# MiNeves00/SR-GAN-FD

Hardware: AMD Instinct MI355X
Metric: SR training images/sec (128->512 x4, f16) (higher is better)
Workload: dtype f16; 1 GPU; BSRGAN RRDBNet x4 generator-only (L1), 23 RRDB, batch 32/GPU, 128->512; global_batch=32, num_rrdb=23, parallelism=dp1

## Files before the change

include/srganfd.h:

```cpp
#ifndef SRGANFD_H
#define SRGANFD_H
#include <stddef.h>
#include <stdint.h>
#ifdef __cplusplus
extern "C" {
#endif

#define SRGANFD_OK 0
#define SRGANFD_EINVAL (-1)
#define SRGANFD_EHIP (-2)
#define SRGANFD_ENOSPC (-3)

#define SRGANFD_BF16 0
#define SRGANFD_F32 1
#define SRGANFD_F16 2

#define SRGANFD_ACT_NONE 0
#define SRGANFD_ACT_LRELU 1
#define SRGANFD_ACT_RELU 2

const char* srganfd_last_error(void);
#define SRGANFD_ABI_VERSION 7
int srganfd_abi_version(void);
void srganfd_set_dry_run(int on);
// ... 26 lines not shown
  srganfd_view y2;
  int32_t out_classes, class_pad_step;
} srganfd_conv_args;

int srganfd_conv2d(const srganfd_conv_args* a, void* stream);
int srganfd_conv2d_describe(const srganfd_conv_args* a, char* out, size_t out_len);

int srganfd_dense_chain(const srganfd_conv_args* layers, int32_t n_layers, void* workspace, size_t workspace_bytes, void* stream);
int srganfd_dense_chain_check(const srganfd_conv_args* layers, int32_t n_layers);
size_t srganfd_dense_chain_workspace_bytes(void);

typedef struct {
  int64_t src_off;
  int64_t scale_off;
  int32_t co_src, ci_src;
  int32_t k_lo, k_len;
  int32_t co_off, ci_off;
  int32_t transposed;
  float scale;
} srganfd_pack_seg;

typedef struct {
  int64_t dst_off;
  int32_t dtype, ksize;
  int32_t k, n;
  int32_t nseg;
  int32_t layout;
  srganfd_pack_seg seg[5];
} srganfd_pack_job;

size_t srganfd_packed_bytes(int32_t dtype, int32_t ksize, int32_t k, int32_t n);
int srganfd_get_mfma16(void);
int srganfd_pack_layout(int32_t dtype, int32_t ksize, int32_t n);
int srganfd_pack_weights(const srganfd_pack_job* jobs_dev, int32_t njobs, int64_t max_elems,
                         const float* params, const float* scalars, void* packed, void* stream);

typedef struct {
  int32_t ci_lo, cin;
  int32_t co_lo, cout;
  int64_t dw_off;
  int64_t db_off;
  int32_t co_dst, ci_dst;
  float alpha;
  float beta;
  int64_t alpha_off;
} srganfd_wgrad_conv;

typedef struct {
  int32_t dtype;
  int32_t n, h_in, w_in, up, ksize, stride, pad, h_out, w_out;
  int32_t x_channels, dy_channels;
  int32_t nconv;
  int32_t splits;
} srganfd_wgrad_shape;

size_t srganfd_wgrad_plan_bytes(const srganfd_wgrad_shape* s, const srganfd_wgrad_conv* convs);
int srganfd_wgrad_plan_build(const srganfd_wgrad_shape* s, const srganfd_wgrad_conv* convs,
                             void* plan_host, size_t plan_bytes, size_t* workspace_bytes);
int srganfd_conv2d_wgrad(const void* plan_host, const void* plan_dev, srganfd_view x, srganfd_view dy,
                         float* grads, const float* scalars, void* workspace, size_t workspace_bytes,
                         void* stream);
typedef struct {
  const void* plan_host; const void* plan_dev;
  float* grads; const float* scalars; const void* workspace;
} srganfd_wgrad_reduce_job;
int srganfd_conv2d_wgrad_partial(const void* plan_host, const void* plan_dev, srganfd_view x, srganfd_view dy,
                                 void* workspace, size_t workspace_bytes, void* stream);
int srganfd_wgrad_reduce_batch(const srganfd_wgrad_reduce_job* jobs, int32_t njobs, void* stream);

int srganfd_nchw_to_nhwc(const float* src, int32_t n, int32_t c, int32_t h, int32_t w, srganfd_view dst,
                         int32_t dtype, int32_t cpad, const float* ch_mean, const float* ch_std, void* stream);
int srganfd_nhwc_to_nchw(srganfd_view src, int32_t dtype, int32_t n, int32_t c, int32_t h, int32_t w,
                         float* dst, int32_t clamp01, void* stream);
int srganfd_clamp_grad_to_nhwc(const float* dsr_nchw, srganfd_view pre_f32, int32_t n, int32_t c, int32_t h,
                               int32_t w, srganfd_view dst, int32_t dtype, int32_t cpad, void* stream);

int srganfd_resample(int32_t op, srganfd_view a, srganfd_view b, int32_t dtype, int32_t n, int32_t h,
                     int32_t w, int32_t c, void* stream);
int srganfd_resample_bwd_lrelu(srganfd_view dy, srganfd_view dx_raw, srganfd_view act, srganfd_view dx_masked,
                               int32_t dtype, int32_t n, int32_t h, int32_t w, int32_t c, float slope, void* stream);
int srganfd_lrelu_bwd(srganfd_view dy, srganfd_view act, srganfd_view skip, srganfd_view out, int32_t dtype,
                      int64_t npix, int32_t c, float slope, void* stream);
int srganfd_axpby(srganfd_view x, srganfd_view y, int32_t dtype, int64_t npix, int32_t c, float alpha,
                  float beta, void* stream);

#define SRGANFD_LOSS_WS_FLOATS 2049
int srganfd_l1_loss(const float* a, const float* b, int64_t numel, float weight, float* out,
                    int32_t accumulate, float* grad_a , float grad_scale,
                    const float* grad_scale_dev , float* workspace, void* stream);
int srganfd_l1_loss_views(srganfd_view a, srganfd_view b, int32_t dtype, int64_t npix, int32_t c,
                          int32_t relu_first, float weight, float* out, int32_t accumulate,
                          float* workspace, void* stream);
int srganfd_bce_logits(const float* logits, int64_t numel, float target, float weight, float* loss_out,
                       int32_t accumulate, float* sigmoid_mean_out , float* grad ,
                       float grad_scale, const float* grad_scale_dev , float* workspace, void* stream);
int srganfd_bce_logits_relativistic(const float* x, int64_t numel, const float* other, int64_t numel_other, float target, float weight,
                                    float* loss_out, int32_t accumulate, float* grad_x , int32_t accumulate_x,
                                    float* grad_other , int32_t accumulate_other, float grad_scale,
                                    const float* grad_scale_dev , float* workspace, void* stream);
int srganfd_sigmoid_of_mean(const float* logits, int64_t numel, float* out, float* workspace, void* stream);

int srganfd_spectral_norm(const float* w_orig, float* u, float* v, int32_t rows, int32_t cols,
                          int32_t training, float eps, float* sigma_out, float* inv_sigma_out,
                          float* workspace, void* stream);
#define SRGANFD_SN_BATCH 8
typedef struct srganfd_sn_job {
  const float* w_orig; float* u; float* v; float* sigma_out; float* inv_sigma_out; float* workspace;
  int32_t rows, cols;
} srganfd_sn_job;
int srganfd_spectral_norm_batch(const srganfd_sn_job* jobs, int32_t njobs, int32_t training, float eps, void* stream);
int srganfd_spectral_norm_grad(const float* g_weight, const float* w_orig, const float* u, const float* v,
                               const float* inv_sigma, float* dw_orig, int32_t rows, int32_t cols,
                               float beta, float* workspace, void* stream);
typedef struct srganfd_sn_grad_job {
  const float* g_weight; const float* w_orig; const float* u; const float* v; const float* inv_sigma;
  float* dw_orig; float* workspace;
  int32_t rows, cols;
} srganfd_sn_grad_job;
int srganfd_spectral_norm_grad_batch(const srganfd_sn_grad_job* jobs, int32_t njobs, float beta, void* stream);

int srganfd_adam_ema(float* param, const float* grad, float* exp_avg, float* exp_avg_sq, float* ema,
// ... 167 lines not shown
```

sr_gan_fd_amd/_abi.py:

```python
from __future__ import annotations

import ctypes as C
import os

_HERE = os.path.dirname(os.path.abspath(__file__))
LIB_PATH = os.environ.get("SRGANFD_LIB") or os.path.join(_HERE, "libsrganfd_hip.so")

HEADER = os.path.join(os.path.dirname(_HERE), "include", "srganfd.h")


_ABI_VERSION_BUILT = 7


def _header_abi_version() -> int:
    import re
    try:
        with open(HEADER) as f:
            m = re.search(r"^#define\s+SRGANFD_ABI_VERSION\s+(\d+)", f.read(), re.M)
    except OSError:
        return _ABI_VERSION_BUILT
    if not m:
        raise RuntimeError(f"{HEADER}: SRGANFD_ABI_VERSION not found")
    return int(m.group(1))

# ... 99 lines not shown
    ]


class LpipsTap(C.Structure):
    C_NAME = "srganfd_lpips_tap"
    _fields_ = [("maps", C.c_void_p), ("lin", C.c_void_p), ("h", C.c_int32), ("w", C.c_int32), ("c", C.c_int32), ("pad_", C.c_int32)]


class AttnArgs(C.Structure):
    C_NAME = "srganfd_attn_args"
    _fields_ = [
        ("dtype", C.c_int32), ("batch", C.c_int32), ("seq", C.c_int32), ("heads", C.c_int32), ("head_dim", C.c_int32), ("pad_", C.c_int32),
        ("qkv", C.c_void_p), ("out", C.c_void_p), ("lse", C.c_void_p), ("d_out", C.c_void_p), ("d_qkv", C.c_void_p), ("weights", C.c_void_p),
        ("workspace", C.c_void_p), ("workspace_bytes", C.c_size_t),
    ]


SYMBOLS = {
    "srganfd_last_error": (C.c_char_p, []),
    "srganfd_abi_version": (C.c_int, []),
    "srganfd_set_dry_run": (None, [C.c_int]),
    "srganfd_get_mfma16": (C.c_int, []),
    "srganfd_pack_layout": (C.c_int, [C.c_int32, C.c_int32, C.c_int32]),
    "srganfd_conv2d": (C.c_int, [C.POINTER(ConvArgs), C.c_void_p]),
    "srganfd_conv2d_describe": (C.c_int, [C.POINTER(ConvArgs), C.c_char_p, C.c_size_t]),
    "srganfd_dense_chain": (C.c_int, [C.POINTER(ConvArgs), C.c_int32, C.c_void_p, C.c_size_t, C.c_void_p]),
    "srganfd_dense_chain_check": (C.c_int, [C.POINTER(ConvArgs), C.c_int32]),
    "srganfd_dense_chain_workspace_bytes": (C.c_size_t, []),
    "srganfd_conv2d_thin_in": (C.c_int, [C.POINTER(ThinArgs), C.c_void_p]),
    "srganfd_conv2d_thin_out": (C.c_int, [C.POINTER(ThinArgs), C.c_void_p]),
    "srganfd_conv2d_thin_wgrad_workspace": (C.c_size_t, []),
    "srganfd_conv2d_thin_wgrad": (C.c_int, [C.POINTER(ThinArgs), C.c_void_p, C.c_void_p, C.c_void_p, C.c_size_t, C.c_void_p]),
    "srganfd_packed_bytes": (C.c_size_t, [C.c_int32, C.c_int32, C.c_int32, C.c_int32]),
    "srganfd_pack_weights": (C.c_int, [C.c_void_p, C.c_int32, C.c_int64, C.c_void_p, C.c_void_p, C.c_void_p, C.c_void_p]),
    "srganfd_wgrad_plan_bytes": (C.c_size_t, [C.POINTER(WgradShape), C.POINTER(WgradConv)]),
    "srganfd_wgrad_plan_build": (C.c_int, [C.POINTER(WgradShape), C.POINTER(WgradConv), C.c_void_p, C.c_size_t,
                                           C.POINTER(C.c_size_t)]),
    "srganfd_conv2d_wgrad_partial": (C.c_int, [C.c_void_p, C.c_void_p, View, View, C.c_void_p, C.c_size_t, C.c_void_p]),
    "srganfd_wgrad_reduce_batch": (C.c_int, [C.c_void_p, C.c_int32, C.c_void_p]),
    "srganfd_conv2d_wgrad": (C.c_int, [C.c_void_p, C.c_void_p, View, View, C.c_void_p, C.c_void_p, C.c_void_p,
                                       C.c_size_t, C.c_void_p]),
    "srganfd_nchw_to_nhwc": (C.c_int, [C.c_void_p, C.c_int32, C.c_int32, C.c_int32, C.c_int32, View, C.c_int32, C.c_int32, C.c_void_p, C.c_void_p, C.c_void_p]),
    "srganfd_lrelu_bwd": (C.c_int, [View, View, View, View, C.c_int32, C.c_int64, C.c_int32, C.c_float, C.c_void_p]),
    "srganfd_nhwc_to_nchw": (C.c_int, [View, C.c_int32, C.c_int32, C.c_int32, C.c_int32, C.c_int32, C.c_void_p, C.c_int32, C.c_void_p]),
    "srganfd_clamp_grad_to_nhwc": (C.c_int, [C.c_void_p, View, C.c_int32, C.c_int32, C.c_int32, C.c_int32, View, C.c_int32, C.c_int32, C.c_void_p]),
    "srganfd_resample_bwd_lrelu": (C.c_int, [View, View, View, View, C.c_int32, C.c_int32, C.c_int32, C.c_int32, C.c_int32, C.c_float, C.c_void_p]),
    "srganfd_resample": (C.c_int, [C.c_int32, View, View, C.c_int32, C.c_int32, C.c_int32, C.c_int32, C.c_int32, C.c_void_p]),
    "srganfd_axpby": (C.c_int, [View, View, C.c_int32, C.c_int64, C.c_int32, C.c_float, C.c_float, C.c_void_p]),
    "srganfd_l1_loss": (C.c_int, [C.c_void_p, C.c_void_p, C.c_int64, C.c_float, C.c_void_p, C.c_int32, C.c_void_p, C.c_float, C.c_void_p, C.c_void_p, C.c_void_p]),
    "srganfd_l1_loss_views": (C.c_int, [View, View, C.c_int32, C.c_int64, C.c_int32, C.c_int32, C.c_float, C.c_void_p, C.c_int32, C.c_void_p, C.c_void_p]),
    "srganfd_sigmoid_of_mean": (C.c_int, [C.c_void_p, C.c_int64, C.c_void_p, C.c_void_p, C.c_void_p]),
    "srganfd_bce_logits": (C.c_int, [C.c_void_p, C.c_int64, C.c_float, C.c_float, C.c_void_p, C.c_int32, C.c_void_p, C.c_void_p, C.c_float, C.c_void_p, C.c_void_p, C.c_void_p]),
    "srganfd_bce_logits_relativistic": (C.c_int, [C.c_void_p, C.c_int64, C.c_void_p, C.c_int64, C.c_float, C.c_float, C.c_void_p, C.c_int32, C.c_void_p, C.c_int32,
                                                  C.c_void_p, C.c_int32, C.c_float, C.c_void_p, C.c_void_p, C.c_void_p]),
    "srganfd_spectral_norm": (C.c_int, [C.c_void_p, C.c_void_p, C.c_void_p, C.c_int32, C.c_int32, C.c_int32, C.c_float, C.c_void_p, C.c_void_p, C.c_void_p, C.c_void_p]),
    "srganfd_spectral_norm_grad": (C.c_int, [C.c_void_p, C.c_void_p, C.c_void_p, C.c_void_p, C.c_void_p, C.c_void_p, C.c_int32, C.c_int32, C.c_float, C.c_void_p, C.c_void_p]),
    "srganfd_spectral_norm_batch": (C.c_int, [C.c_void_p, C.c_int32, C.c_int32, C.c_float, C.c_void_p]),
    "srganfd_spectral_norm_grad_batch": (C.c_int, [C.c_void_p, C.c_int32, C.c_float, C.c_void_p]),
    "srganfd_adam_ema": (C.c_int, [C.c_void_p, C.c_void_p, C.c_void_p, C.c_void_p, C.c_void_p, C.c_int64, C.c_float, C.c_float, C.c_float, C.c_float,
                                   C.c_float, C.c_int32, C.c_float, C.c_float, C.c_int32, C.c_void_p, C.c_void_p, C.c_void_p]),
    "srganfd_loss_scale_update": (C.c_int, [C.c_void_p, C.c_void_p, C.c_float, C.c_float, C.c_int32, C.c_void_p]),
    "srganfd_nonfinite_flag": (C.c_int, [C.c_void_p, C.c_int64, C.c_void_p, C.c_int32, C.c_void_p]),
    "srganfd_resize_bilinear": (C.c_int, [C.c_int32, View, View, C.c_int32, C.c_int32, C.c_int32, C.c_int32, C.c_int32, C.c_int32, C.c_int32, C.c_void_p]),
    "srganfd_add_relu": (C.c_int, [View, View, View, C.c_int32, C.c_int64, C.c_int32, C.c_void_p]),
    "srganfd_sigmoid": (C.c_int, [C.c_void_p, C.c_int64, C.c_void_p]),
    "srganfd_sigmoid_bwd": (C.c_int, [C.c_void_p, C.c_void_p, C.c_void_p, C.c_int64, C.c_void_p]),
    "srganfd_adam_ema_dev": (C.c_int, [C.c_void_p, C.c_void_p, C.c_void_p, C.c_void_p, C.c_void_p, C.c_int64, C.c_float, C.c_float, C.c_float, C.c_float,
                                       C.c_float, C.c_void_p, C.c_void_p, C.c_float, C.c_float, C.c_int32, C.c_void_p, C.c_void_p, C.c_void_p]),
    "srganfd_l1_grad_views": (C.c_int, [View, View, View, C.c_int32, C.c_int64, C.c_int32, C.c_void_p, C.c_float, C.c_void_p]),
    "srganfd_maxpool2_relu_bwd": (C.c_int, [View, View, View, C.c_int32, C.c_int32, C.c_int32, C.c_int32, C.c_int32, C.c_void_p]),
    "srganfd_nhwc_to_nchw_scaled": (C.c_int, [View, C.c_int32, C.c_int32, C.c_int32, C.c_int32, C.c_void_p, C.c_void_p, C.c_void_p]),
    "srganfd_crop_nchw": (C.c_int, [C.c_void_p, C.c_void_p] + [C.c_int32] * 8 + [C.c_void_p]),
    "srganfd_u8hwc_to_nchw": (C.c_int, [C.c_void_p, C.c_void_p] + [C.c_int32] * 8 + [C.c_float, C.c_void_p]),
    "srganfd_psnr": (C.c_int, [C.c_void_p, C.c_void_p] + [C.c_int32] * 6 + [C.c_void_p, C.c_void_p, C.c_void_p]),
    "srganfd_filter2d": (C.c_int, [C.c_void_p, C.c_void_p] + [C.c_int32] * 6 + [C.c_void_p, C.c_void_p]),
    "srganfd_filter2d_separable": (C.c_int, [C.c_void_p, C.c_void_p] + [C.c_int32] * 6 + [C.c_void_p, C.c_void_p]),
    "srganfd_usm_sharp": (C.c_int, [C.c_void_p, C.c_void_p] + [C.c_int32] * 6 + [C.c_float, C.c_float, C.c_void_p, C.c_void_p, C.c_void_p]),
    "srganfd_diff_jpeg_table_floats": (C.c_int32, []),
    "srganfd_diff_jpeg_tables": (C.c_int, [C.c_void_p]),
    "srganfd_diff_jpeg": (C.c_int, [C.c_void_p] + [C.c_int32] * 4 + [C.c_void_p, C.c_int32, C.c_int32, C.c_void_p, C.c_void_p, C.c_void_p]),
    "srganfd_jpeg_workspace_bytes": (C.c_int64, [C.c_int32] * 3),
    "srganfd_jpeg_roundtrip": (C.c_int, [C.c_void_p] + [C.c_int32] * 4 + [C.c_void_p] * 5),
# ... 106 lines not shown
```

sr_gan_fd_amd/csrc/loss.hip:

```cpp
#include "elementwise.hpp"

namespace srganfd {

__global__ __launch_bounds__(256) void l1_partial_kernel(const float* __restrict__ a, const float* __restrict__ b, size_t n, float gscale,
                                                         const float* __restrict__ gscale_dev, float* __restrict__ grad, float* __restrict__ partial) {
  __shared__ float sh[4];
  float s = 0.f;
  if (gscale_dev) gscale *= *gscale_dev;
  for (size_t i = (size_t)blockIdx.x * 256 + threadIdx.x; i < n; i += (size_t)gridDim.x * 256) {
    const float d = a[i] - b[i];
    s += fabsf(d);
    if (grad) grad[i] = d > 0.f ? gscale : (d < 0.f ? -gscale : 0.f);
  }
  const float r = block_reduce_sum(s, sh);
  if (threadIdx.x == 0) partial[blockIdx.x] = r;
}
template <typename T>
__global__ __launch_bounds__(256) void l1_views_partial_kernel(const void* __restrict__ a, int aC, int a0, const void* __restrict__ b, int bC, int b0,
                                                               size_t npix, int c, int relu, float* __restrict__ partial) {
  __shared__ float sh[4];
  float s = 0.f;
  const size_t total = npix * c;
  for (size_t i = (size_t)blockIdx.x * 256 + threadIdx.x; i < total; i += (size_t)gridDim.x * 256) {
    const int ch = (int)(i % c);
    const size_t p = i / c;
    float va = ld<T>(a, p * aC + a0 + ch), vb = ld<T>(b, p * bC + b0 + ch);
    if (relu) { va = fmaxf(va, 0.f); vb = fmaxf(vb, 0.f); }
    s += fabsf(va - vb);
  }
  const float r = block_reduce_sum(s, sh);
  if (threadIdx.x == 0) partial[blockIdx.x] = r;
}
template <typename T>
__global__ __launch_bounds__(256) void l1_views_vec_partial_kernel(const void* __restrict__ a, int aC, int a0, const void* __restrict__ b, int bC, int b0,
                                                                   size_t npix, int c, int relu, float* __restrict__ partial) {
  constexpr int N = VecN<T>::N;
  __shared__ float sh[4];
  float s = 0.f;
  const int cv = c / N;
  const size_t total = npix * cv;
  for (size_t i = (size_t)blockIdx.x * 256 + threadIdx.x; i < total; i += (size_t)gridDim.x * 256) {
    const int ch = (int)(i % cv) * N;
    const size_t p = i / cv;
    float va[N], vb[N];
    ldv<T>(a, p * aC + a0 + ch, va);
// ... 112 lines not shown
  if (__any(bad) && (threadIdx.x & 63) == 0) *flag = 1.f;
}

__global__ void loss_scale_update_kernel(float* __restrict__ st, const float* __restrict__ found_inf, float growth, float backoff, int interval) {
  if (threadIdx.x != 0 || blockIdx.x != 0) return;
  int* sti = reinterpret_cast<int*>(st);
  float scale = st[0];
  int tracker = sti[2];
  sti[3] += 1;
  if (*found_inf != 0.f) {
    scale *= backoff; tracker = 0; sti[4] += 1;
  } else {
    tracker += 1;
    if (tracker >= interval) {
      const float grown = scale * growth;
      if (fabsf(grown) <= 3.402823466e38f) scale = grown;
      tracker = 0;
    }
  }
  st[0] = scale; st[1] = 1.f / scale; sti[2] = tracker;
}

extern "C" int srganfd_l1_loss(const float* a, const float* b, int64_t numel, float weight, float* out, int32_t accumulate, float* grad, float grad_scale,
                               const float* grad_scale_dev, float* ws, void* stream) {
  const size_t n = (size_t)numel;
  const hipStream_t s = (hipStream_t)stream;
  if (!a || !b || !out || !ws || n == 0) return set_err(SRGANFD_EINVAL, "l1_loss: bad args");
  const unsigned g = grid_for(n, 256, kRedBlocks);
  SRGANFD_LAUNCH(l1_partial_kernel, dim3(g), dim3(256), 0, s, a, b, n, grad_scale / (float)n, grad_scale_dev, grad, ws);
  SRGANFD_LAUNCH(finish_sum_kernel, dim3(1), dim3(256), 0, s, (const float*)ws, (int)g, weight / (float)n, out, accumulate);
  SRGANFD_HIP_CHECK(hipGetLastError());
  return SRGANFD_OK;
}
extern "C" int srganfd_l1_loss_views(srganfd_view a, srganfd_view b, int32_t dtype, int64_t npix64, int32_t c, int32_t relu, float weight, float* out,
                                     int32_t accumulate, float* ws, void* stream) {
  const size_t npix = (size_t)npix64;
  const hipStream_t s = (hipStream_t)stream;
  if (!a.ptr || !b.ptr || !out || !ws) return set_err(SRGANFD_EINVAL, "l1_views: bad args");
  const size_t n = npix * c;
  const unsigned g = grid_for(n, 256, kRedBlocks);
  const int vn = dtype == SRGANFD_F32 ? 4 : 8;
  if (c % vn == 0 && a.c0 % vn == 0 && b.c0 % vn == 0 && a.cstride % vn == 0 && b.cstride % vn == 0 && ((uintptr_t)a.ptr & 15) == 0 && ((uintptr_t)b.ptr & 15) == 0) {
    DISPATCH_T(dtype,
               SRGANFD_LAUNCH(l1_views_vec_partial_kernel<TT>, dim3(g), dim3(256), 0, s, a.ptr, a.cstride, a.c0, b.ptr, b.cstride, b.c0, npix, c, relu, ws));
  } else
  DISPATCH_T(dtype,
             SRGANFD_LAUNCH(l1_views_partial_kernel<TT>, dim3(g), dim3(256), 0, s, a.ptr, a.cstride, a.c0, b.ptr, b.cstride, b.c0, npix, c, relu, ws));
  SRGANFD_LAUNCH(finish_sum_kernel, dim3(1), dim3(256), 0, s, (const float*)ws, (int)g, weight / (float)n, out, accumulate);
  SRGANFD_HIP_CHECK(hipGetLastError());
  return SRGANFD_OK;
}
extern "C" int srganfd_l1_grad_views(srganfd_view a, srganfd_view b, srganfd_view out, int32_t dtype, int64_t npix64, int32_t c, const float* upstream,
                                     float scale, void* stream) {
  const size_t npix = (size_t)npix64;
  const hipStream_t s = (hipStream_t)stream;
  if (!a.ptr || !b.ptr || !out.ptr || npix == 0 || c <= 0) return set_err(SRGANFD_EINVAL, "l1_grad_views: bad args");
  DISPATCH_T(dtype,
             SRGANFD_LAUNCH(l1_grad_views_kernel<TT>, dim3(grid_for(npix * c)), dim3(256), 0, s, a.ptr, a.cstride, a.c0, b.ptr, b.cstride, b.c0, out.ptr, out.cstride, out.c0, npix, c, upstream, scale));
  SRGANFD_HIP_CHECK(hipGetLastError());
  return SRGANFD_OK;
}
extern "C" int srganfd_bce_logits(const float* x, int64_t numel, float target, float weight, float* loss_out, int32_t accumulate, float* sig_mean_out,
                                  float* grad, float grad_scale, const float* grad_scale_dev, float* ws, void* stream) {
  const size_t n = (size_t)numel;
  const hipStream_t s = (hipStream_t)stream;
  if (!x || !loss_out || !ws || n == 0) return set_err(SRGANFD_EINVAL, "bce: bad args");
// ... 55 lines not shown
```

sr_gan_fd_amd/csrc/pack.hip:

```cpp
#include "common.hpp"

namespace srganfd {

__global__ __launch_bounds__(256) void pack_kernel(const srganfd_pack_job* __restrict__ jobs, const float* __restrict__ params,
                                                   const float* __restrict__ scalars, char* __restrict__ packed) {
  const srganfd_pack_job& J = jobs[blockIdx.y];
  const int KT = J.ksize * J.ksize;
  const long long total = (long long)KT * J.k * J.n;
  const int nChunks = J.k >> 5;
  for (long long e = (long long)blockIdx.x * 256 + threadIdx.x; e < total; e += (long long)gridDim.x * 256) {
    int lane, s, k_in, within = (int)(e & 1023);
    long long blk = e >> 10;
    const int tap = (int)(blk % KT); blk /= KT;
    const int chunk = (int)(blk % nChunks);
    const int ntile = (int)(blk / nChunks);
    int n_in = -1;
    if (J.dtype != SRGANFD_F32 && J.layout == 1) {
      const int j = within & 7; lane = (within >> 3) & 63; s = within >> 9;
      k_in = 8 * (lane >> 4) + j;
      n_in = 16 * s + (lane & 15);
    } else if (J.dtype != SRGANFD_F32) {
      const int j = within & 7; lane = (within >> 3) & 63; s = within >> 9;
      k_in = 16 * s + 8 * (lane >> 5) + j;
    } else {
      lane = within & 63; s = within >> 6;
      k_in = 2 * s + (lane >> 5);
    }
    const int k = chunk * 32 + k_in, n = ntile * 32 + (n_in >= 0 ? n_in : (lane & 31));
    float v = 0.f;
    for (int g = 0; g < J.nseg; ++g) {
      const srganfd_pack_seg& S = J.seg[g];
      if (k >= S.k_lo && k < S.k_lo + S.k_len) {
        const int kk = k - S.k_lo;
        int co, ci, t = 0;
        int KTs = KT;
        int ym = 0, xm = 0;
        if (!S.transposed) { co = n + S.co_off; ci = kk + S.ci_off; t = tap; }
        else if (S.transposed == 1) { co = kk + S.co_off; ci = n + S.ci_off; t = KT - 1 - tap; }
        else if (S.transposed < 6) {
          const int py = (S.transposed - 2) >> 1, px = (S.transposed - 2) & 1, ta = tap >> 1, tb = tap & 1;
          const int ty = py ? 2 - 2 * ta : 3 - 2 * ta, tx = px ? 2 - 2 * tb : 3 - 2 * tb;
          co = kk + S.co_off; ci = n + S.ci_off; t = ty * 4 + tx; KTs = 16;
        } else if (S.transposed < 10) {
// ... 2 lines not shown
          co = kk + S.co_off; ci = n + S.ci_off; KTs = 9;
          t = ty * 3 + tx;
          if (ty < 0 || tx < 0) co = S.co_src;
        } else if (S.transposed < 14) {
          const int ab = S.transposed - 10;
          co = kk + S.co_off; ci = n + S.ci_off; t = ab; KTs = 4;
        } else if (S.transposed < 18) {
          const int py = (S.transposed - 14) >> 1, px = (S.transposed - 14) & 1, ta = tap >> 1, tb = tap & 1;
          co = n + S.co_off; ci = kk + S.ci_off; KTs = 9;
          ym = py ? (ta ? 4 : 3) : (ta ? 6 : 1);
          xm = px ? (tb ? 4 : 3) : (tb ? 6 : 1);
        } else {
          const int u = tap >> 2, w = tap & 3;
          co = kk + S.co_off; ci = n + S.ci_off; KTs = 9;
          ym = (0x1364 >> (4 * u)) & 7;
          xm = (0x1364 >> (4 * w)) & 7;
        }
        if (co < S.co_src && ci < S.ci_src) {
          const float* src = params + S.src_off + ((long long)co * S.ci_src + ci) * KTs;
          if (ym) {
            float sum = 0.f;
            for (int ty = 0; ty < 3; ++ty)
              for (int tx = 0; tx < 3; ++tx)
                if ((ym >> ty) & (xm >> tx) & 1) sum += src[ty * 3 + tx];
            v = sum * S.scale;
          } else {
            v = src[t] * S.scale;
          }
          if (S.scale_off >= 0) v *= scalars[S.scale_off];
        }
        break;
      }
    }
    if (J.dtype == SRGANFD_BF16) ((bf16_t*)(packed + J.dst_off))[e] = f2bf(v);
    else if (J.dtype == SRGANFD_F16) ((f16_t*)(packed + J.dst_off))[e] = (f16_t)v;
    else ((float*)(packed + J.dst_off))[e] = v;
  }
}

extern "C" size_t srganfd_packed_bytes(int32_t dtype, int32_t ksize, int32_t k, int32_t n) {
  if (k <= 0 || n <= 0 || k % 32 || n % 32) return 0;
  return (size_t)ksize * ksize * k * n * (dtype == SRGANFD_F32 ? 4 : 2);
}
extern "C" int srganfd_pack_weights(const srganfd_pack_job* jobs_dev, int32_t njobs, int64_t max_elems, const float* params,
                                    const float* scalars, void* packed, void* stream) {
  if (!jobs_dev || njobs <= 0 || max_elems <= 0 || !params || !packed) return set_err(SRGANFD_EINVAL, "pack_weights: bad args");
  long long gx = (max_elems + 255) / 256;
  if (gx > 4096) gx = 4096;
  SRGANFD_LAUNCH(pack_kernel, dim3((unsigned)gx, (unsigned)njobs), dim3(256), 0, (hipStream_t)stream, jobs_dev, params, scalars, (char*)packed);
  SRGANFD_HIP_CHECK(hipGetLastError());
  return SRGANFD_OK;
}

}
```

sr_gan_fd_amd/engine.py:

```python
from __future__ import annotations

import ctypes as C
import os
import weakref
from typing import Dict, List, Optional, Sequence, Tuple

import torch
from torch import Tensor, nn

from . import _abi as A
from . import ops
from . import profiling

_ENGINES: "weakref.WeakKeyDictionary[nn.Module, object]" = weakref.WeakKeyDictionary()


def _require_gpu(x: Tensor) -> None:
    if not x.is_cuda and not A.DRY_RUN:
        raise A.SrganfdError("sr_gan_fd_amd runs on MI355X only: input tensor is not on a GPU (no CPU fallback)")
    A.lib()


def check_channels(what: str, x: Tensor, channels: int) -> None:
    if x.dim() != 4 or x.shape[1] != channels:
# ... 401 lines not shown
                bw.extend(chain[:4] + [wg] + ready + fence + chain[4:])
        if self.full:
            bw.append(ops.Call("srganfd_axpby", (V(sp.d_f0), V(sp.dx0), dtc, N * H * W, Cc, 1.0, 1.0), "axpby"))
            bw.append(ops.image_wgrad(dtc, sp.thin_i, wplans, sp.xin, sp.dx0, fptr + 4 * self._poff("conv1.weight"), self._poff("conv1.weight"),
                                      self._poff("conv1.bias"), sp.thin_ws, N, H, W, self.in_ch, Cc, True))
        covered = min([it.payload[0] for it in bw if it.kind == "ready"], default=self.fp.total)
        bw.append(ops.Item("ready", (0, covered)))
        sp.bw = bw
        sp.wg_ws = wplans.workspace()
        dense_ws = max((p_.workspace_bytes for p_ in plans.values()), default=0)
        sp.wg_ws4 = [torch.empty(dense_ws, dtype=torch.uint8, device=device) for _ in range(_BATCH_REDUCE)] if (dense_ws and _BATCH_REDUCE > 1) else None

    def trunk_size(self, shape) -> Tuple[int, int, int]:
        shape = tuple(shape)
        u = self.unshuffle
        want_c = self.in_ch // (u * u) if self.full else self.Cc
        what = "generator" if self.full else "dense block"
        if len(shape) != 4:
            raise A.SrganfdError(f"{what} expects a 4-D (N, {want_c}, H, W) input, got shape {shape}")
        N, c, H, W = shape
        if c != want_c:
            raise A.SrganfdError(f"{what} expects (N, {want_c}, H, W) inputs, got shape {shape}")
        if H % u or W % u:
            raise A.SrganfdError(f"generator with PixelUnshuffle({u}) expects H and W divisible by {u}: (N, {want_c}, {u}k, {u}m), "
                                 f"got shape {shape}")
        return N, H // u, W // u

    def output_shape(self, shape) -> Tuple[int, int, int, int]:
        N, H, W = self.trunk_size(shape)
        if not self.full:
            return (N, self.Cc, H, W)
        return (N, self.out_ch, H << self.n_up, W << self.n_up)

    def forward(self, x: Tensor, train: bool) -> Tensor:
        N, H, W = self.trunk_size(x.shape)
        _require_gpu(x)
        dt, dtc = _dt(self.owner)
        dev = x.device
        pk = self._ensure_packed(dtc, dev)
        sp = self._plan(N, H, W, dt, dtc, dev, train, pk)
        if self.unshuffle > 1:
            x = torch.nn.functional.pixel_unshuffle(x, self.unshuffle)
        x = x.contiguous().float()
        L, st = A.lib(), A.stream_ptr()
        if self.full:
            A.check(L.srganfd_nchw_to_nhwc(x.data_ptr(), N, self.in_ch, H, W, A.view(sp.xin), dtc, sp.xin.shape[-1], None, None, st), "nchw_to_nhwc")
        else:
            A.check(L.srganfd_nchw_to_nhwc(x.data_ptr(), N, self.Cc, H, W, A.view(sp.catb(0)), dtc, self.Cc, None, None, st), "nchw_to_nhwc")
        rec = profiling.REC
        for item in sp.fw:
            if item.kind == "conv":
                ops.conv2d(item.args, rec, "conv2d", L, st)
            else:
                item.launch(rec, L, st)
        if self.full:
            out = torch.empty(N, self.out_ch, sp.hs, sp.ws, dtype=torch.float32, device=dev)
            A.check(L.srganfd_nhwc_to_nchw(A.view(sp.srp), A.F32, N, self.out_ch, sp.hs, sp.ws, out.data_ptr(), 1, st), "nhwc_to_nchw")
        else:
            out = torch.empty(N, self.Cc, H, W, dtype=torch.float32, device=dev)
            A.check(L.srganfd_nhwc_to_nchw(A.view(sp.catb(self.R)), dtc, N, self.Cc, H, W, out.data_ptr(), 0, st), "nhwc_to_nchw")
        if train:
            self.token += 1
            sp.token = self.token
        self._last = sp
        return out

    def backward(self, sp: _Shape, token: int, dout: Tensor, need_dx: bool, on_ready=None) -> Tuple[Tensor, Optional[Tensor]]:
        if getattr(sp, "token", None) != token:
            raise A.SrganfdError("generator activations were overwritten by a later training-mode forward before backward ran")
        L, st = A.lib(), A.stream_ptr()
        N, H, W, dtc = sp.N, sp.H, sp.W, sp.dtc
        dout = dout.contiguous().float()
        flat_grad = self.fp.new_grad(sp.device)
        if self.full:
            A.check(L.srganfd_clamp_grad_to_nhwc(dout.data_ptr(), A.view(sp.srp), N, self.out_ch, sp.hs, sp.ws, A.view(sp.dsrp), dtc, sp.dsrp.shape[-1], st), "clamp_grad")
        else:
            A.check(L.srganfd_nchw_to_nhwc(dout.data_ptr(), N, self.Cc, H, W, A.view(sp.dy[(self.R - 1) % 4]), dtc, self.Cc, None, None, st), "nchw_to_nhwc")
        gptr = flat_grad.data_ptr()
        rec = profiling.REC
        pend_red = []
        side = None
        if _WGRAD_STREAM and sp.wg_ws4 is not None:
            side = getattr(sp, "wg_stream", None)
            if side is None:
                side = sp.wg_stream = torch.cuda.Stream(device=sp.device)
            main = torch.cuda.current_stream()
            wg_done = {}

        def on_side(fn):
            if side is None:
                return fn()
            with torch.cuda.stream(side):
                return fn()

        def flush_reduce():
            if not pend_red:
                return
            jobs = (A.WgradReduceJob * len(pend_red))()
            for j, (plan, goff, ws) in zip(jobs, pend_red):
                j.plan_host, j.plan_dev = C.addressof(plan.host), plan.dev.data_ptr()
                j.grads, j.scalars, j.workspace = gptr + 4 * goff, None, ws.data_ptr()
            n_jobs = len(pend_red)
            run = lambda: A.check(L.srganfd_wgrad_reduce_batch(jobs, n_jobs, A.stream_ptr()), "wgrad_reduce_batch")
            on_side(run if rec is None else lambda: rec.bracket("wgrad_reduce_batch", (0.0, float(sum(w.numel() for _, _, w in pend_red))), run))
            pend_red.clear()
        for item in sp.bw:
            kind = item.kind
# ... 112 lines not shown
```

sr_gan_fd_amd/trainer.py:

```python
from __future__ import annotations

from typing import Dict, Optional, Tuple

import torch
from torch import Tensor

from . import _abi as A
from .engine import generator_engine
from .parallel import BucketReducer, allreduce_sum_


class LossScaler:

    def __init__(self, device, enabled: bool = True, init_scale: float = 65536.0, growth_factor: float = 2.0, backoff_factor: float = 0.5,
                 growth_interval: int = 2000):
        self.enabled = enabled
        self.growth_factor, self.backoff_factor, self.growth_interval = growth_factor, backoff_factor, growth_interval
        if enabled:
            self.state = torch.zeros(8, dtype=torch.float32, device=device)
            self.state[0] = float(init_scale)
            self.state[1] = 1.0 / float(init_scale)
            self.flag = torch.zeros(1, dtype=torch.float32, device=device)

    @property
    def seed_ptr(self):
        return self.state.data_ptr() if self.enabled else None

    @property
    def inv_ptr(self):
        return self.state.data_ptr() + 4 if self.enabled else None

    @property
    def scale(self) -> float:
        return float(self.state[0].item()) if self.enabled else 1.0
# ... 248 lines not shown
            return
        A.check(A.lib().srganfd_adam_ema(self.flat.data_ptr(), grad.data_ptr(), self.m.data_ptr(), self.v.data_ptr(),
                                         self.ema.data_ptr() if self.ema is not None else None, self.flat.numel(), self.lr,
                                         self.betas[0], self.betas[1], self.eps, self.wd, self.t, grad_scale,
                                         self.ema_decay or 0.0, mode, None, grad_scale_dev, A.stream_ptr()), "adam_ema")


class GanCheckpointMixin:

    def state_dict(self) -> dict:
        g = {"state_dict": self.g.state_dict(), "optimizer": self.g_opt.state_dict()}
        if self.g_opt.ema is not None:
            g["ema_state_dict"] = self.g_opt.ema_state_dict()
        return {"g": g, "d": {"state_dict": self.d.state_dict(), "optimizer": self.d_opt.state_dict()}, "scaler": self.scaler.state_dict()}

    def load_state_dict(self, ckpt: dict) -> None:
        with torch.no_grad():
            for net, eng, opt, c in ((self.g, self.ge, self.g_opt, ckpt.get("g")), (self.d, self.de, self.d_opt, ckpt.get("d"))):
                if c is None:
                    continue
                own = net.state_dict()
                for k, v in c["state_dict"].items():
                    if k in own and tuple(own[k].shape) == tuple(v.shape):
                        own[k].copy_(v)
                eng.fp.touch()
                if "optimizer" in c:
                    opt.load_state_dict(c["optimizer"])
                if "ema_state_dict" in c and opt.ema is not None:
                    opt.load_ema_state_dict(c["ema_state_dict"])
        if "scaler" in ckpt:
            self.scaler.load_state_dict(ckpt["scaler"])


class GeneratorTrainer:

    def __init__(self, g_model, lr: float, betas=(0.9, 0.99), eps: float = 1e-8, weight_decay: float = 0.0,
                 ema_decay: Optional[float] = 0.999, loss_weight: float = 1.0, process_group=None):
        self.g = g_model
        pin_training_dtype(g_model)
        self.eng = generator_engine(g_model)
        dev = next(g_model.parameters()).device
        self.flat = self.eng.fp.sync(dev)
        self.opt = FlatAdamEMA(self.flat, lr, betas, eps, weight_decay, ema_decay, layout=self.eng.fp)
        self.loss_weight = loss_weight
        self.scaler = LossScaler(dev, enabled=needs_loss_scaling(g_model))
        self.pg = process_group
        self.g_reducer = BucketReducer(dev, process_group)
        self.loss_buf = torch.zeros(1, dtype=torch.float32, device=dev)
        self.ws = torch.empty(A.LOSS_WS_FLOATS, dtype=torch.float32, device=dev)
        self.dsr: Optional[Tensor] = None

    def state_dict(self) -> dict:
        out = {"state_dict": self.g.state_dict(), "optimizer": self.opt.state_dict()}
        if self.opt.ema is not None:
            out["ema_state_dict"] = self.opt.ema_state_dict()
        return out

    def load_state_dict(self, ckpt: dict) -> None:
        with torch.no_grad():
            own = self.g.state_dict()
            for k, v in ckpt["state_dict"].items():
                if k in own and tuple(own[k].shape) == tuple(v.shape):
                    own[k].copy_(v)
        self.eng.fp.touch()
        if "optimizer" in ckpt:
            self.opt.load_state_dict(ckpt["optimizer"])
        if "ema_state_dict" in ckpt and self.opt.ema is not None:
            self.opt.load_ema_state_dict(ckpt["ema_state_dict"])

    def step(self, lr_img: Tensor, gt: Tensor) -> Tensor:
        eng = self.eng
        check_targets("GeneratorTrainer.step", eng, lr_img, gt=gt)
        sr = eng.forward(lr_img, True)
        sp, token = eng._last, eng.token
        if self.dsr is None or self.dsr.shape != sr.shape:
            self.dsr = torch.empty_like(sr)
        gt = gt.contiguous().float()
        check_loss_scaling(self.scaler, self.g)
        A.check(A.lib().srganfd_l1_loss(sr.data_ptr(), gt.data_ptr(), sr.numel(), self.loss_weight, self.loss_buf.data_ptr(), 0,
                                        self.dsr.data_ptr(), self.loss_weight, self.scaler.seed_ptr, self.ws.data_ptr(), A.stream_ptr()), "l1_loss")
        self.g_reducer.begin()
        grad, _ = eng.backward(sp, token, self.dsr, False, on_ready=self.g_reducer.bucket)
        scale = self.g_reducer.finish()
        self.scaler.step(self.opt, grad, scale)
        eng.fp.touch()
        self.sr = sr
        return self.loss_buf
```

Before: 539.4 img/s.

## Add fused one-pass L1 loss head and tiled weight-pack kernel

Adds a fused kernel that clamps the fp32 NHWC pre-activation, writes the NCHW SR output, computes the L1 loss and writes the masked 16-bit NHWC gradient in a single pass. This replaces the separate nhwc_to_nchw, l1_loss and clamp_grad kernels, but it sits behind SRGANFD_FUSED_L1_HEAD, which is off by default. It also adds a tiled weight-packing kernel, enabled by default, that stages weight rows through shared memory with vectorized loads before emitting the packed layout. That aims to cut per-element index math and uncoalesced reads in the per-step repack, at the cost of more complex code paths per transpose mode.

```diff
diff --git a/include/srganfd.h b/include/srganfd.h
--- a/include/srganfd.h
+++ b/include/srganfd.h
@@ -82,6 +82,7 @@
 size_t srganfd_packed_bytes(int32_t dtype, int32_t ksize, int32_t k, int32_t n);
 int srganfd_get_mfma16(void);
 int srganfd_pack_layout(int32_t dtype, int32_t ksize, int32_t n);
+int srganfd_set_pack_tiled(int32_t on);
 int srganfd_pack_weights(const srganfd_pack_job* jobs_dev, int32_t njobs, int64_t max_elems,
                          const float* params, const float* scalars, void* packed, void* stream);
 
@@ -137,6 +138,9 @@
 #define SRGANFD_LOSS_WS_FLOATS 2049
 int srganfd_l1_loss(const float* a, const float* b, int64_t numel, float weight, float* out,
                     int32_t accumulate, float* grad_a , float grad_scale,
+                    const float* grad_scale_dev , float* workspace, void* stream);
+int srganfd_l1_head(srganfd_view pre_f32, const float* gt_nchw, int32_t n, int32_t c, int32_t h, int32_t w,
+                    float* sr_nchw, srganfd_view dgrad, int32_t dtype, float weight, float* out, float grad_scale,
                     const float* grad_scale_dev , float* workspace, void* stream);
 int srganfd_l1_loss_views(srganfd_view a, srganfd_view b, int32_t dtype, int64_t npix, int32_t c,
                           int32_t relu_first, float weight, float* out, int32_t accumulate,
diff --git a/sr_gan_fd_amd/_abi.py b/sr_gan_fd_amd/_abi.py
--- a/sr_gan_fd_amd/_abi.py
+++ b/sr_gan_fd_amd/_abi.py
@@ -155,6 +155,7 @@
     "srganfd_conv2d_thin_wgrad_workspace": (C.c_size_t, []),
     "srganfd_conv2d_thin_wgrad": (C.c_int, [C.POINTER(ThinArgs), C.c_void_p, C.c_void_p, C.c_void_p, C.c_size_t, C.c_void_p]),
     "srganfd_packed_bytes": (C.c_size_t, [C.c_int32, C.c_int32, C.c_int32, C.c_int32]),
+    "srganfd_set_pack_tiled": (C.c_int, [C.c_int32]),
     "srganfd_pack_weights": (C.c_int, [C.c_void_p, C.c_int32, C.c_int64, C.c_void_p, C.c_void_p, C.c_void_p, C.c_void_p]),
     "srganfd_wgrad_plan_bytes": (C.c_size_t, [C.POINTER(WgradShape), C.POINTER(WgradConv)]),
     "srganfd_wgrad_plan_build": (C.c_int, [C.POINTER(WgradShape), C.POINTER(WgradConv), C.c_void_p, C.c_size_t,
@@ -171,6 +172,8 @@
     "srganfd_resample": (C.c_int, [C.c_int32, View, View, C.c_int32, C.c_int32, C.c_int32, C.c_int32, C.c_int32, C.c_void_p]),
     "srganfd_axpby": (C.c_int, [View, View, C.c_int32, C.c_int64, C.c_int32, C.c_float, C.c_float, C.c_void_p]),
     "srganfd_l1_loss": (C.c_int, [C.c_void_p, C.c_void_p, C.c_int64, C.c_float, C.c_void_p, C.c_int32, C.c_void_p, C.c_float, C.c_void_p, C.c_void_p, C.c_void_p]),
+    "srganfd_l1_head": (C.c_int, [View, C.c_void_p, C.c_int32, C.c_int32, C.c_int32, C.c_int32, C.c_void_p, View, C.c_int32, C.c_float, C.c_void_p, C.c_float,
+                                  C.c_void_p, C.c_void_p, C.c_void_p]),
     "srganfd_l1_loss_views": (C.c_int, [View, View, C.c_int32, C.c_int64, C.c_int32, C.c_int32, C.c_float, C.c_void_p, C.c_int32, C.c_void_p, C.c_void_p]),
     "srganfd_sigmoid_of_mean": (C.c_int, [C.c_void_p, C.c_int64, C.c_void_p, C.c_void_p, C.c_void_p]),
     "srganfd_bce_logits": (C.c_int, [C.c_void_p, C.c_int64, C.c_float, C.c_float, C.c_void_p, C.c_int32, C.c_void_p, C.c_void_p, C.c_float, C.c_void_p, C.c_void_p, C.c_void_p]),
diff --git a/sr_gan_fd_amd/csrc/loss.hip b/sr_gan_fd_amd/csrc/loss.hip
--- a/sr_gan_fd_amd/csrc/loss.hip
+++ b/sr_gan_fd_amd/csrc/loss.hip
@@ -11,6 +11,33 @@
     const float d = a[i] - b[i];
     s += fabsf(d);
     if (grad) grad[i] = d > 0.f ? gscale : (d < 0.f ? -gscale : 0.f);
+  }
+  const float r = block_reduce_sum(s, sh);
+  if (threadIdx.x == 0) partial[blockIdx.x] = r;
+}
+template <typename T>
+__global__ __launch_bounds__(256) void l1_head_rgb4_kernel(const f32x4* __restrict__ pre, const float* __restrict__ gt, float* __restrict__ sr,
+                                                           unsigned long long* __restrict__ dst, size_t npix, size_t hw, int c, float gscale,
+                                                           const float* __restrict__ gscale_dev, float* __restrict__ partial) {
+  __shared__ float sh[4];
+  float s = 0.f;
+  if (gscale_dev) gscale *= *gscale_dev;
+  for (size_t p = (size_t)blockIdx.x * 256 + threadIdx.x; p < npix; p += (size_t)gridDim.x * 256) {
+    const size_t img = p / hw, pix = p % hw;
+    const f32x4 q = pre[p];
+    float v[8] = {0.f, 0.f, 0.f, 0.f, 0.f, 0.f, 0.f, 0.f};
+#pragma unroll
+    for (int k = 0; k < 4; ++k)
+      if (k < c) {
+        const size_t i = (img * c + k) * hw + pix;
+        const float a = q[k] < 0.f ? 0.f : (q[k] > 1.f ? 1.f : q[k]);
+        sr[i] = a;
+        const float d = a - gt[i];
+        s += fabsf(d);
+        if (q[k] >= 0.f && q[k] <= 1.f) v[k] = d > 0.f ? gscale : (d < 0.f ? -gscale : 0.f);
+      }
+    const u32x4 w0 = pack8<T>(v);
+    dst[p] = (unsigned long long)w0[0] | ((unsigned long long)w0[1] << 32);
   }
   const float r = block_reduce_sum(s, sh);
   if (threadIdx.x == 0) partial[blockIdx.x] = r;
@@ -189,6 +216,26 @@
   SRGANFD_HIP_CHECK(hipGetLastError());
   return SRGANFD_OK;
 }
+extern "C" int srganfd_l1_head(srganfd_view pre, const float* gt, int32_t n, int32_t c, int32_t h, int32_t w, float* sr, srganfd_view dgrad, int32_t dtype,
+                               float weight, float* out, float grad_scale, const float* grad_scale_dev, float* ws, void* stream) {
+  const hipStream_t s = (hipStream_t)stream;
+  if (!pre.ptr || !gt || !sr || !dgrad.ptr || !out || !ws || n <= 0 || c <= 0 || h <= 0 || w <= 0) return set_err(SRGANFD_EINVAL, "l1_head: bad args");
+  if (pre.planar || dgrad.planar) return set_err(SRGANFD_EINVAL, "l1_head: NHWC views only, not planar ones");
+  if ((dtype != SRGANFD_BF16 && dtype != SRGANFD_F16) || c > 4 || pre.cstride != 4 || pre.c0 != 0 || dgrad.cstride != 4 || dgrad.c0 != 0 ||
+      ((uintptr_t)pre.ptr & 15) || ((uintptr_t)dgrad.ptr & 7))
+    return set_err(SRGANFD_EINVAL, "l1_head: needs an fp32 4-channel pre-clamp view and a 16-bit 4-channel gradient view (c <= 4), both whole and aligned");
+  const size_t npix = (size_t)n * h * w, numel = npix * c;
+  const unsigned g = grid_for(npix, 256, 2 * kRedBlocks);
+  if (dtype == SRGANFD_BF16)
+    SRGANFD_LAUNCH(l1_head_rgb4_kernel<bf16_t>, dim3(g), dim3(256), 0, s, (const f32x4*)pre.ptr, gt, sr, (unsigned long long*)dgrad.ptr, npix, (size_t)h * w, c,
+                   grad_scale / (float)numel, grad_scale_dev, ws);
+  else
+    SRGANFD_LAUNCH(l1_head_rgb4_kernel<f16_t>, dim3(g), dim3(256), 0, s, (const f32x4*)pre.ptr, gt, sr, (unsigned long long*)dgrad.ptr, npix, (size_t)h * w, c,
+                   grad_scale / (float)numel, grad_scale_dev, ws);
+  SRGANFD_LAUNCH(finish_sum_kernel, dim3(1), dim3(256), 0, s, (const float*)ws, (int)g, weight / (float)numel, out, 0);
+  SRGANFD_HIP_CHECK(hipGetLastError());
+  return SRGANFD_OK;
+}
 extern "C" int srganfd_l1_loss_views(srganfd_view a, srganfd_view b, int32_t dtype, int64_t npix64, int32_t c, int32_t relu, float weight, float* out,
                                      int32_t accumulate, float* ws, void* stream) {
   const size_t npix = (size_t)npix64;
diff --git a/sr_gan_fd_amd/csrc/pack.hip b/sr_gan_fd_amd/csrc/pack.hip
--- a/sr_gan_fd_amd/csrc/pack.hip
+++ b/sr_gan_fd_amd/csrc/pack.hip
@@ -1,14 +1,10 @@
 #include "common.hpp"
+#include <stdlib.h>
 
 namespace srganfd {
 
-__global__ __launch_bounds__(256) void pack_kernel(const srganfd_pack_job* __restrict__ jobs, const float* __restrict__ params,
-                                                   const float* __restrict__ scalars, char* __restrict__ packed) {
-  const srganfd_pack_job& J = jobs[blockIdx.y];
-  const int KT = J.ksize * J.ksize;
-  const long long total = (long long)KT * J.k * J.n;
-  const int nChunks = J.k >> 5;
-  for (long long e = (long long)blockIdx.x * 256 + threadIdx.x; e < total; e += (long long)gridDim.x * 256) {
+__device__ __forceinline__ float pack_element(const srganfd_pack_job& J, const int KT, const int nChunks, const long long e,
+                                              const float* __restrict__ params, const float* __restrict__ scalars) {
     int lane, s, k_in, within = (int)(e & 1023);
     long long blk = e >> 10;
     const int tap = (int)(blk % KT); blk /= KT;
@@ -77,12 +73,194 @@
         break;
       }
     }
+    return v;
+}
+__device__ __forceinline__ void pack_store(const srganfd_pack_job& J, char* __restrict__ packed, const long long e, const float v) {
     if (J.dtype == SRGANFD_BF16) ((bf16_t*)(packed + J.dst_off))[e] = f2bf(v);
     else if (J.dtype == SRGANFD_F16) ((f16_t*)(packed + J.dst_off))[e] = (f16_t)v;
     else ((float*)(packed + J.dst_off))[e] = v;
-  }
-}
-
+}
+__global__ __launch_bounds__(256) void pack_kernel(const srganfd_pack_job* __restrict__ jobs, const float* __restrict__ params,
+                                                   const float* __restrict__ scalars, char* __restrict__ packed) {
+  const srganfd_pack_job& J = jobs[blockIdx.y];
+  const int KT = J.ksize * J.ksize;
+  const long long total = (long long)KT * J.k * J.n;
+  const int nChunks = J.k >> 5;
+  for (long long e = (long long)blockIdx.x * 256 + threadIdx.x; e < total; e += (long long)gridDim.x * 256)
+    pack_store(J, packed, e, pack_element(J, KT, nChunks, e, params, scalars));
+}
+
+#ifndef SRGANFD_PACK_BATCH
+#define SRGANFD_PACK_BATCH 4
+#endif
+static constexpr int kPackTileFloats = 32 * (32 * 9 + 1);
+
+__device__ __forceinline__ void pack_tap(const int tr, const int KT, const int tap, int& t, bool& ok) {
+  t = 0; ok = true;
+  if (!tr) t = tap;
+  else if (tr == 1) t = KT - 1 - tap;
+  else if (tr < 6) {
+    const int py = (tr - 2) >> 1, px = (tr - 2) & 1, ta = tap >> 1, tb = tap & 1;
+    const int ty = py ? 2 - 2 * ta : 3 - 2 * ta, tx = px ? 2 - 2 * tb : 3 - 2 * tb;
+    t = ty * 4 + tx;
+  } else if (tr < 10) {
+    const int py = (tr - 6) >> 1, px = (tr - 6) & 1, ta = tap >> 1, tb = tap & 1;
+    const int ty = py ? (ta ? 0 : 2) : (ta ? -1 : 1), tx = px ? (tb ? 0 : 2) : (tb ? -1 : 1);
+    ok = !(ty < 0 || tx < 0);
+    t = ok ? ty * 3 + tx : 0;
+  } else t = tr - 10;
+}
+
+struct PackTile {
+  int KT, KTs, RS;
+  int rows, pass;
+  int rvalid, cvalid;
+  float scale, scale2;
+};
+
+template <int LAY, bool BF, bool FO, bool CHECK>
+__device__ __forceinline__ void pack_produce(const float* __restrict__ tile, const unsigned* __restrict__ tapinfo, const PackTile P, char* __restrict__ dst) {
+  constexpr bool JR = (LAY < 2) != FO;
+  const int stride = JR ? P.RS : P.KTs;
+  for (int gi = threadIdx.x; gi < P.KT * 128; gi += 256) {
+    const int tap = gi >> 7, q = gi & 127;
+    int kb, nb;
+    if (LAY == 2) { kb = 2 * (q >> 3) + ((q & 7) >> 2); nb = (8 * (q & 7)) & 31; }
+    else if (LAY == 1) { const int lane = q & 63; kb = 8 * (lane >> 4); nb = 16 * (q >> 6) + (lane & 15); }
+    else { const int lane = q & 63; kb = 16 * (q >> 6) + 8 * (lane >> 5); nb = lane & 31; }
+    const int r0 = FO ? nb : kb, c0 = FO ? kb : nb;
+    if (P.rows < 32 && (r0 >> 4) != P.pass) continue;
+    const unsigned info = tapinfo[tap];
+    const int t = info & 0xff;
+    const bool ok = (info >> 16) & 1;
+    const int idx0 = (r0 - P.pass * P.rows) * P.RS + c0 * P.KTs + t;
+    float v[8];
+#pragma unroll
+    for (int j = 0; j < 8; ++j) {
+      const bool valid = !CHECK || (ok && (r0 + (JR ? j : 0) < P.rvalid) && (c0 + (JR ? 0 : j) < P.cvalid));
+      const float x = tile[valid ? idx0 + j * stride : 0];
+      v[j] = valid ? x : 0.f;
+    }
+    if (LAY == 2) {
+      const f32x4 a = {v[0], v[1], v[2], v[3]}, b = {v[4], v[5], v[6], v[7]};
+      f32x4* o = (f32x4*)dst + 2 * gi;
+      o[0] = a; o[1] = b;
+    } else {
+      ((u32x4*)dst)[gi] = BF ? pack8<bf16_t>(v) : pack8<f16_t>(v);
+    }
+  }
+}
+
+__global__ __launch_bounds__(256) void pack_tiled_kernel(const srganfd_pack_job* __restrict__ jobs, const float* __restrict__ params,
+                                                         const float* __restrict__ scalars, char* __restrict__ packed) {
+  __shared__ float tile[kPackTileFloats];
+  __shared__ unsigned tapinfo[16];
+  const srganfd_pack_job& J = jobs[gridDim.y - 1 - blockIdx.y];
+  const int KT = J.ksize * J.ksize, nChunks = J.k >> 5, nUnits = nChunks * (J.n >> 5);
+  bool sums = false;
+  for (int i = 0; i < J.nseg; ++i) sums |= J.seg[i].transposed >= 14;
+  if (sums) {
+    const long long total = (long long)KT * J.k * J.n;
+    for (long long e = (long long)blockIdx.x * 256 + threadIdx.x; e < total; e += (long long)gridDim.x * 256)
+      pack_store(J, packed, e, pack_element(J, KT, nChunks, e, params, scalars));
+    return;
+  }
+  const int dtype = J.dtype, lay = dtype == SRGANFD_F32 ? 2 : (J.layout == 1 ? 1 : 0);
+  for (int unit = blockIdx.x; unit < nUnits; unit += gridDim.x) {
+    const int ntile = unit / nChunks, chunk = unit - ntile * nChunks, k0 = chunk * 32;
+    const long long ebase = (long long)unit * KT * 1024;
+    int g = -1;
+    for (int i = 0; i < J.nseg; ++i) {
+      const srganfd_pack_seg& Q = J.seg[i];
+      if (Q.k_lo < k0 + 32 && Q.k_lo + Q.k_len > k0) {
+        if (k0 >= Q.k_lo && k0 + 32 <= Q.k_lo + Q.k_len) g = i;
+        break;
+      }
+    }
+    if (g < 0) {
+      for (int i = threadIdx.x; i < KT * 1024; i += 256) pack_store(J, packed, ebase + i, pack_element(J, KT, nChunks, ebase + i, params, scalars));
+      continue;
+    }
+    const srganfd_pack_seg& S = J.seg[g];
+    const int tr = S.transposed, co_src = S.co_src, ci_src = S.ci_src;
+    const bool fo = tr == 0;
+    PackTile P;
+    P.KT = KT;
+    P.KTs = tr < 2 ? KT : (tr < 6 ? 16 : (tr < 10 ? 9 : 4));
+    P.RS = 32 * P.KTs + 1;
+    P.rows = 32 * P.RS <= kPackTileFloats ? 32 : 16;
+    const int kk0 = k0 - S.k_lo;
+    const int co0 = (fo ? ntile * 32 : kk0) + S.co_off, ci0 = (fo ? kk0 : ntile * 32) + S.ci_off;
+    P.rvalid = co_src - co0; P.cvalid = ci_src - ci0;
+    P.scale = S.scale; P.scale2 = S.scale_off >= 0 ? scalars[S.scale_off] : 1.f;
+    const bool bf = dtype == SRGANFD_BF16;
+    const int len = P.cvalid <= 0 ? 0 : (P.cvalid < 32 ? P.cvalid : 32) * P.KTs;
+    const bool check = P.rvalid < 32 || P.cvalid < 32 || (tr >= 6 && tr < 10);
+    const float* tbase = params + S.src_off + ((long long)co0 * ci_src + ci0) * P.KTs;
+    char* dst = packed + J.dst_off + ebase * (lay == 2 ? 4 : 2);
+    for (P.pass = 0; P.pass * P.rows < 32; ++P.pass) {
+      __syncthreads();
+      if (P.pass == 0 && threadIdx.x < KT) {
+        int t; bool ok;
+        pack_tap(tr, KT, threadIdx.x, t, ok);
+        tapinfo[threadIdx.x] = (unsigned)t | ((unsigned)ok << 16);
+      }
+      {
+        const int lpr = 256 / P.rows;
+        const int rr = threadIdx.x / lpr, l = threadIdx.x - rr * lpr, row = P.pass * P.rows + rr;
+        if (row < P.rvalid && len > 0) {
+          const float* rowp = tbase + (long long)row * ci_src * P.KTs;
+          const int mis = (int)(((uintptr_t)rowp >> 2) & 3);
+          const f32x4* vp = (const f32x4*)(rowp - mis);
+          const int nvec = (mis + len + 3) >> 2;
+          float* trow = tile + rr * P.RS;
+          constexpr int kBatch = SRGANFD_PACK_BATCH;
+          for (int v0 = l; v0 < nvec; v0 += kBatch * lpr) {
+            f32x4 x[kBatch];
+#pragma unroll
+            for (int i = 0; i < kBatch; ++i)
+              if (v0 + i * lpr < nvec) x[i] = vp[v0 + i * lpr];
+#pragma unroll
+            for (int i = 0; i < kBatch; ++i) {
+              const int j0 = 4 * (v0 + i * lpr) - mis;
+              if (v0 + i * lpr >= nvec) continue;
+              if (j0 >= 0 && j0 + 3 < len) {
+                trow[j0] = x[i][0] * P.scale * P.scale2; trow[j0 + 1] = x[i][1] * P.scale * P.scale2;
+                trow[j0 + 2] = x[i][2] * P.scale * P.scale2; trow[j0 + 3] = x[i][3] * P.scale * P.scale2;
+              } else {
+#pragma unroll
+                for (int q = 0; q < 4; ++q)
+                  if (j0 + q >= 0 && j0 + q < len) trow[j0 + q] = x[i][q] * P.scale * P.scale2;
+              }
+            }
+          }
+        }
+      }
+      __syncthreads();
+#define SRGANFD_PACK_PRODUCE(LAY, BF) \
+      if (fo) { if (check) pack_produce<LAY, BF, true, true>(tile, tapinfo, P, dst); else pack_produce<LAY, BF, true, false>(tile, tapinfo, P, dst); } \
+      else { if (check) pack_produce<LAY, BF, false, true>(tile, tapinfo, P, dst); else pack_produce<LAY, BF, false, false>(tile, tapinfo, P, dst); }
+      if (lay == 2) { SRGANFD_PACK_PRODUCE(2, false) }
+      else if (lay == 1) { if (bf) { SRGANFD_PACK_PRODUCE(1, true) } else { SRGANFD_PACK_PRODUCE(1, false) } }
+      else { if (bf) { SRGANFD_PACK_PRODUCE(0, true) } else { SRGANFD_PACK_PRODUCE(0, false) } }
+#undef SRGANFD_PACK_PRODUCE
+    }
+  }
+}
+
+static int g_pack_tiled = -1;
+static int pack_tiled() {
+  if (g_pack_tiled < 0) {
+    const char* e = getenv("SRGANFD_PACK_TILED");
+    g_pack_tiled = !(e && e[0] == '0' && !e[1]);
+  }
+  return g_pack_tiled;
+}
+extern "C" int srganfd_set_pack_tiled(int32_t on) {
+  const int was = pack_tiled();
+  if (on >= 0) g_pack_tiled = on ? 1 : 0;
+  return was;
+}
 extern "C" size_t srganfd_packed_bytes(int32_t dtype, int32_t ksize, int32_t k, int32_t n) {
   if (k <= 0 || n <= 0 || k % 32 || n % 32) return 0;
   return (size_t)ksize * ksize * k * n * (dtype == SRGANFD_F32 ? 4 : 2);
@@ -90,6 +268,13 @@
 extern "C" int srganfd_pack_weights(const srganfd_pack_job* jobs_dev, int32_t njobs, int64_t max_elems, const float* params,
                                     const float* scalars, void* packed, void* stream) {
   if (!jobs_dev || njobs <= 0 || max_elems <= 0 || !params || !packed) return set_err(SRGANFD_EINVAL, "pack_weights: bad args");
+  if (pack_tiled() && ((uintptr_t)packed & 15) == 0) {
+    long long gx = (max_elems + 9 * 1024 - 1) / (9 * 1024);
+    if (gx > 65535) gx = 65535;
+    SRGANFD_LAUNCH(pack_tiled_kernel, dim3((unsigned)gx, (unsigned)njobs), dim3(256), 0, (hipStream_t)stream, jobs_dev, params, scalars, (char*)packed);
+    SRGANFD_HIP_CHECK(hipGetLastError());
+    return SRGANFD_OK;
+  }
   long long gx = (max_elems + 255) / 256;
   if (gx > 4096) gx = 4096;
   SRGANFD_LAUNCH(pack_kernel, dim3((unsigned)gx, (unsigned)njobs), dim3(256), 0, (hipStream_t)stream, jobs_dev, params, scalars, (char*)packed);
diff --git a/sr_gan_fd_amd/engine.py b/sr_gan_fd_amd/engine.py
--- a/sr_gan_fd_amd/engine.py
+++ b/sr_gan_fd_amd/engine.py
@@ -457,7 +457,7 @@
             return (N, self.Cc, H, W)
         return (N, self.out_ch, H << self.n_up, W << self.n_up)
 
-    def forward(self, x: Tensor, train: bool) -> Tensor:
+    def forward(self, x: Tensor, train: bool, to_pre: bool = False) -> Optional[Tensor]:
         N, H, W = self.trunk_size(x.shape)
         _require_gpu(x)
         dt, dtc = _dt(self.owner)
@@ -478,7 +478,9 @@
                 ops.conv2d(item.args, rec, "conv2d", L, st)
             else:
                 item.launch(rec, L, st)
-        if self.full:
+        if to_pre and train and self.l1_head_ok(sp):
+            out = None
+        elif self.full:
             out = torch.empty(N, self.out_ch, sp.hs, sp.ws, dtype=torch.float32, device=dev)
             A.check(L.srganfd_nhwc_to_nchw(A.view(sp.srp), A.F32, N, self.out_ch, sp.hs, sp.ws, out.data_ptr(), 1, st), "nhwc_to_nchw")
         else:
@@ -490,14 +492,24 @@
         self._last = sp
         return out
 
-    def backward(self, sp: _Shape, token: int, dout: Tensor, need_dx: bool, on_ready=None) -> Tuple[Tensor, Optional[Tensor]]:
+    def l1_head_ok(self, sp: _Shape) -> bool:
+        dsrp = getattr(sp, "dsrp", None)
+        return bool(self.full and getattr(sp, "thin_o", False) and dsrp is not None and dsrp.shape[-1] == 4 and self.out_ch <= 4)
+
+    def backward(self, sp: _Shape, token: int, dout: Optional[Tensor], need_dx: bool, on_ready=None) -> Tuple[Tensor, Optional[Tensor]]:
         if getattr(sp, "token", None) != token:
             raise A.SrganfdError("generator activations were overwritten by a later training-mode forward before backward ran")
         L, st = A.lib(), A.stream_ptr()
         N, H, W, dtc = sp.N, sp.H, sp.W, sp.dtc
-        dout = dout.contiguous().float()
+        if dout is None:
+            if not self.l1_head_ok(sp):
+                raise A.SrganfdError("backward(dout=None) needs a generator plan whose sp.dsrp the one-pass L1 head has written")
+        else:
+            dout = dout.contiguous().float()
         flat_grad = self.fp.new_grad(sp.device)
-        if self.full:
+        if dout is None:
+            pass
+        elif self.full:
             A.check(L.srganfd_clamp_grad_to_nhwc(dout.data_ptr(), A.view(sp.srp), N, self.out_ch, sp.hs, sp.ws, A.view(sp.dsrp), dtc, sp.dsrp.shape[-1], st), "clamp_grad")
         else:
             A.check(L.srganfd_nchw_to_nhwc(dout.data_ptr(), N, self.Cc, H, W, A.view(sp.dy[(self.R - 1) % 4]), dtc, self.Cc, None, None, st), "nchw_to_nhwc")
diff --git a/sr_gan_fd_amd/trainer.py b/sr_gan_fd_amd/trainer.py
--- a/sr_gan_fd_amd/trainer.py
+++ b/sr_gan_fd_amd/trainer.py
@@ -1,5 +1,6 @@
 from __future__ import annotations
 
+import os
 from typing import Dict, Optional, Tuple
 
 import torch
@@ -314,6 +315,9 @@
             self.scaler.load_state_dict(ckpt["scaler"])
 
 
+_FUSED_L1_HEAD = os.environ.get("SRGANFD_FUSED_L1_HEAD", "0") == "1"
+
+
 class GeneratorTrainer:
 
     def __init__(self, g_model, lr: float, betas=(0.9, 0.99), eps: float = 1e-8, weight_decay: float = 0.0,
@@ -353,16 +357,24 @@
     def step(self, lr_img: Tensor, gt: Tensor) -> Tensor:
         eng = self.eng
         check_targets("GeneratorTrainer.step", eng, lr_img, gt=gt)
-        sr = eng.forward(lr_img, True)
+        sr = eng.forward(lr_img, True, to_pre=_FUSED_L1_HEAD)
         sp, token = eng._last, eng.token
-        if self.dsr is None or self.dsr.shape != sr.shape:
-            self.dsr = torch.empty_like(sr)
         gt = gt.contiguous().float()
         check_loss_scaling(self.scaler, self.g)
-        A.check(A.lib().srganfd_l1_loss(sr.data_ptr(), gt.data_ptr(), sr.numel(), self.loss_weight, self.loss_buf.data_ptr(), 0,
-                                        self.dsr.data_ptr(), self.loss_weight, self.scaler.seed_ptr, self.ws.data_ptr(), A.stream_ptr()), "l1_loss")
+        L, st = A.lib(), A.stream_ptr()
+        if sr is None:
+            sr = torch.empty(sp.N, eng.out_ch, sp.hs, sp.ws, dtype=torch.float32, device=sp.device)
+            A.check(L.srganfd_l1_head(A.view(sp.srp), gt.data_ptr(), sp.N, eng.out_ch, sp.hs, sp.ws, sr.data_ptr(), A.view(sp.dsrp), sp.dtc,
+                                      self.loss_weight, self.loss_buf.data_ptr(), self.loss_weight, self.scaler.seed_ptr, self.ws.data_ptr(), st), "l1_head")
+            dsr = None
+        else:
+            if self.dsr is None or self.dsr.shape != sr.shape:
+                self.dsr = torch.empty_like(sr)
+            dsr = self.dsr
+            A.check(L.srganfd_l1_loss(sr.data_ptr(), gt.data_ptr(), sr.numel(), self.loss_weight, self.loss_buf.data_ptr(), 0,
+                                      dsr.data_ptr(), self.loss_weight, self.scaler.seed_ptr, self.ws.data_ptr(), st), "l1_loss")
         self.g_reducer.begin()
-        grad, _ = eng.backward(sp, token, self.dsr, False, on_ready=self.g_reducer.bucket)
+        grad, _ = eng.backward(sp, token, dsr, False, on_ready=self.g_reducer.bucket)
         scale = self.g_reducer.finish()
         self.scaler.step(self.opt, grad, scale)
         eng.fp.touch()
```

After: 540.9 img/s, median of 6. No clear change (+0.3%).
